# qasimyu/simuscop

Hardware: AMD Instinct MI355X
Metric: simulated paired reads/sec (whole node) at 30x WGS PE150 (higher is better)
Workload: dtype u32

## Files before the change

simuscop_amd/csrc/sg_api.cpp:

```cpp
#include <hip/hip_runtime.h>

#include <algorithm>
#include <chrono>
#include <cstdio>
#include <cstdlib>
#include <cstring>
#include <map>
#include <mutex>
#include <string>
#include <vector>

#include "sg_api.h"
#include "sg_deflate.h"
#include "sg_tables.h"
#include "sg_truth.h"

namespace {

struct BlockCache {
  struct Block { void* p; size_t cap; int dev; };
  std::mutex mu;
  std::vector<Block> blocks;
  size_t held = 0;
  static size_t limit() {
// ... 144 lines not shown
  int device = 0;
  hipStream_t stream = nullptr;
  DevBuf text[2], gz[2];
  uint64_t text_bytes[2] = {0, 0}, gz_bytes[2] = {0, 0};
  std::string err;
  ~sg_outputs() {
    if (stream) { (void)hipStreamSynchronize(stream); (void)hipStreamDestroy(stream); }
  }
};

sg_ctx::~sg_ctx() {
  (void)hipSetDevice(device);
  if (stream) (void)hipStreamSynchronize(stream);
  for (sg_outputs* o : spare) delete o;
  if (evs_created)
    for (auto& ev : evs) (void)hipEventDestroy(ev);
  if (own_stream) { (void)hipStreamSynchronize(own_stream); (void)hipStreamDestroy(own_stream); }
  if (mail) (void)hipHostFree(mail);
}

static int finish_plan(sg_ctx* ctx, uint64_t nw, uint32_t n_segs, uint32_t n_slots, uint32_t batch_id, uint32_t first_window,
                       uint32_t first_slot, int32_t paired, const char* name_prefix) {
  const size_t plen = name_prefix ? strlen(name_prefix) : 0;
  const uint32_t nm = paired ? 2 : 1;
  SG_ENSURE(ctx->prefix, plen + 16);
  SG_ENSURE(ctx->pairs, ((size_t)n_slots + 1) * sizeof(sg::PairRec));
  SG_ENSURE(ctx->win_actual, (nw + 1) * 4);
  SG_ENSURE(ctx->win_namebase, (nw + 1) * 4);
  SG_ENSURE(ctx->events, ((size_t)nm * n_slots + 1) * 4 * SG_MAX_EVENTS);
  SG_ENSURE(ctx->recoff, ((size_t)nm * n_slots + 1) * 4);
  SG_ENSURE(ctx->meta, ((size_t)nm * n_slots + 1) * 48);
  SG_ENSURE(ctx->totals, sg::kTotalsBytes);
  SG_ENSURE(ctx->bsum, ((size_t)nm * ((n_slots + 255) / 256) + 1) * 8);
  SG_HIP(hipMemcpyAsync(ctx->prefix.p, name_prefix, plen, hipMemcpyHostToDevice, ctx->stream));
  SG_HIP(hipStreamSynchronize(ctx->stream));

  sg::DevBatch& B = ctx->B;
  B.windows = ctx->windows.as<sg_window>();
  B.n_windows = nw;
  B.seg_size = ctx->segmeta.as<uint32_t>();
  B.seg_first_window = ctx->segmeta.as<uint32_t>() + n_segs;
  B.n_segs = n_segs;
  B.n_slots = n_slots;
  B.batch_id = batch_id;
  B.win_offset = first_window;
  B.slot_offset = first_slot;
  B.paired = paired ? 1 : 0;
  B.prefix = ctx->prefix.as<uint8_t>();
  B.prefix_len = (uint32_t)plen;
  for (int i = 0; i < 4; i++) B.prefix_w[i] = 0;
  for (size_t i = 0; i < plen && i < 16; i++) B.prefix_w[i / 4] |= (uint32_t)(uint8_t)name_prefix[i] << (8 * (i % 4));
  B.pairs = ctx->pairs.as<sg::PairRec>();
  B.win_actual = ctx->win_actual.as<uint32_t>();
  B.win_namebase = ctx->win_namebase.as<uint32_t>();
  B.events = ctx->events.as<uint32_t>();
  B.recloc = ctx->recoff.as<uint32_t>();
  B.blkbase = ctx->bsum.as<uint64_t>();
  B.seg_shift = sg::record_seg_shift((uint32_t)n_slots);
  B.meta = ctx->meta.as<uint4>();
  B.totals = ctx->totals.as<uint64_t>();
  B.slowq_count = (uint32_t*)(B.totals + 4);
  ctx->have_plan = true;
  ctx->sampled = false;
  ctx->results_valid = false;
  return SG_OK;
}

static int pack_chains(sg_ctx* ctx, size_t total) {
  const size_t q = total / 4, badb = total / 64 / 8;
  SG_ENSURE(ctx->chains2, 2 * q + badb + 64);
  uint8_t* p = ctx->chains2.as<uint8_t>();
  sg::launch_pack2(ctx->chains.as<uint8_t>(), total, (uint32_t*)p, (uint32_t*)(p + q), (uint16_t*)(p + 2 * q), ctx->stream);
  ctx->B.chains2_fwd = p;
  ctx->B.chains2_rc = p + q;
  ctx->B.chains_bad = (const uint16_t*)(p + 2 * q);
  ctx->B.chains_total = total;
  return SG_OK;
}

static sg_ctx::ChainLayout chain_layout(int32_t n_chains, const uint64_t* lens) {
  const size_t PAD = 256;
  sg_ctx::ChainLayout L;
  L.len.assign(lens, lens + n_chains);
  L.total = PAD;
  for (int c = 0; c < n_chains; c++) {
    L.off.push_back(L.total);
    L.total += (lens[c] + PAD + 63) & ~(size_t)63;
  }
  L.total = (L.total + PAD + 1023) & ~(size_t)1023;
  return L;
}

static int commit_chains(sg_ctx* ctx, sg_ctx::ChainLayout&& L) {
  std::vector<uint64_t> meta(L.off);
// ... 1010 lines not shown
  if (b->n_segs) {
    SG_HIP(hipMemcpyAsync(ctx->segmeta.p, b->seg_size, (size_t)b->n_segs * 4, hipMemcpyHostToDevice, ctx->stream));
    SG_HIP(hipMemcpyAsync(ctx->segmeta.as<uint32_t>() + b->n_segs, b->seg_first_window, ((size_t)b->n_segs + 1) * 4,
                          hipMemcpyHostToDevice, ctx->stream));
  }
  return finish_plan(ctx, nw, b->n_segs, (uint32_t)slots, b->batch_id, b->first_window, b->first_slot, b->paired, b->name_prefix);
}

static int launch_text(sg_ctx* ctx, bool prof) {
  sg::DevBatch& B = ctx->B;
  hipStream_t s = ctx->stream;
  B.out[0] = ctx->out1.as<uint8_t>();
  B.out[1] = ctx->out2.as<uint8_t>();
  B.out_cap[0] = ctx->out1.cap;
  B.out_cap[1] = ctx->out2.cap;
  B.slowq = nullptr;
  B.slowq_cap = 0;
  if (sg::emit_uses_fast_kernel(ctx->P, B)) {
    uint64_t cap = std::max<uint64_t>(1u << 16, 2ull * B.n_slots);
    if (const char* e = getenv("SG_SLOWQ_CAP")) cap = std::max<uint64_t>(1, strtoull(e, nullptr, 10));
    cap = std::min<uint64_t>(cap, 1ull << 30);
    SG_ENSURE(ctx->slowq, cap * 8 * (B.paired ? 2 : 1));
    B.slowq = ctx->slowq.as<uint2>();
    B.slowq_cap = (uint32_t)cap;
  }
  if (prof) SG_HIP(hipEventRecord(ctx->evs[5], s));
  sg::launch_header(ctx->P, B, s);
  ctx->emit_path = sg::emit_path(ctx->P, B, false);
  sg::launch_emit(ctx->P, B, s, false, prof ? ctx->evs[7] : nullptr);
  if (prof) SG_HIP(hipEventRecord(ctx->evs[6], s));
  return SG_OK;
}

static int run_pass(sg_ctx* ctx) {
  sg::DevBatch& B = ctx->B;
  B.k0 = (uint32_t)ctx->seed;
  B.k1 = (uint32_t)(ctx->seed >> 32);
  { const char* dg = getenv("SG_DIAG"); B.diag = dg ? (uint32_t)atoi(dg) : 0u; }
  if (const char* fd = getenv("SG_FDIAG")) B.diag = (uint32_t)atoi(fd);
  hipStream_t s = ctx->stream;
  const bool prof = ctx->profiling;
  if (!B.n_windows) SG_HIP(hipMemsetAsync(B.totals, 0, sg::kTotalsBytes, s));
  if (prof) SG_HIP(hipEventRecord(ctx->evs[0], s));
  sg::launch_plan(ctx->P, B, s);
  if (prof) SG_HIP(hipEventRecord(ctx->evs[1], s));
  sg::launch_namebase(B, s);
  if (prof) SG_HIP(hipEventRecord(ctx->evs[2], s));
  sg::launch_indel(ctx->P, B, s);
  if (prof) SG_HIP(hipEventRecord(ctx->evs[3], s));
  sg::launch_scan(B, s);
  if (prof) SG_HIP(hipEventRecord(ctx->evs[4], s));
  SG_HIP(hipGetLastError());
  if (!ctx->out1.p && !ctx->out2.p && !ctx->gz1.p && !ctx->gz2.p && !ctx->spare.empty()) {
    sg_outputs* o = ctx->spare.back();
    std::swap(ctx->out1, o->text[0]); std::swap(ctx->out2, o->text[1]);
    std::swap(ctx->gz1, o->gz[0]); std::swap(ctx->gz2, o->gz[1]);
  }
  ctx->speculative = ctx->out1.p != nullptr && (!B.paired || ctx->out2.p != nullptr) && getenv("SG_NO_SPECULATION") == nullptr;
  if (!ctx->speculative) {
    sg::launch_mail(B.totals, ctx->mail, s);
    SG_HIP(hipStreamSynchronize(s));
    memcpy(ctx->host_totals, ctx->mail, 4 * 8);
    if (ctx->host_totals[3] & 1) return ctx->fail(SG_ERR_OVERFLOW, "sg_sample: a read drew more than SG_MAX_EVENTS sequencing indels");
    SG_ENSURE(ctx->out1, ctx->host_totals[0] + 64);
    if (B.paired) SG_ENSURE(ctx->out2, ctx->host_totals[1] + 64);
  }
  if (int rc = launch_text(ctx, prof)) return rc;
  sg::launch_mail(B.totals, ctx->mail, s);
  SG_HIP(hipGetLastError());
  ctx->sampled = true;
  ctx->pass_pending = true;
  ctx->results_valid = false;
  ctx->gz_valid = false;
  return SG_OK;
}

static int finish_pass(sg_ctx* ctx) {
  if (!ctx->pass_pending) return SG_OK;
  SG_HIP(hipStreamSynchronize(ctx->stream));
  ctx->pass_pending = false;
  memcpy(ctx->host_totals, ctx->mail, 4 * 8);
// ... 350 lines not shown
```

simuscop_amd/csrc/sg_api.h:

```cpp
#pragma once
#include <hip/hip_runtime.h>

#include <map>
#include <string>
#include <utility>
#include <vector>

#include "sg_device.h"
#include "sg_haplotypes.h"

struct DevBuf {
  void* p = nullptr;
  size_t cap = 0;
  int dev = 0;
  DevBuf() = default;
  DevBuf(DevBuf&& o) noexcept : p(std::exchange(o.p, nullptr)), cap(std::exchange(o.cap, 0)), dev(o.dev) {}
  DevBuf& operator=(DevBuf&& o) noexcept {
    if (this != &o) { release(); p = std::exchange(o.p, nullptr); cap = std::exchange(o.cap, 0); dev = o.dev; }
    return *this;
  }
  DevBuf(const DevBuf&) = delete;
  DevBuf& operator=(const DevBuf&) = delete;
  ~DevBuf() { release(); }
  int ensure(size_t bytes);
  void release();
  template <class T> T* as() const { return (T*)p; }
};

extern thread_local std::string g_create_error;

struct sg_outputs;
struct sg_train_session;

struct sg_ctx {
  int device = 0;
  hipStream_t own_stream = nullptr;
  hipStream_t stream = nullptr;
  uint64_t seed = 0;
  std::string err;

  bool have_profile = false, have_haps = false, have_plan = false, sampled = false;
  sg::DevProfile P{};
  sg::DevBatch B{};
  DevBuf tab, chains, chains2, chain_meta, windows, segmeta, prefix, pairs, win_actual, win_namebase, events, recoff, meta, totals, bsum,
      out1, out2, gcw, gco, gcm, slowq, ref_raw, ref_codes, ref_meta, hap_work, gz1, gz2, gz_work,
      infl_src, infl_meta, infl_out, infl_crc,
      defl_src, defl_out;
  struct ChainLayout {
    std::vector<uint64_t> off, len;
    size_t total = 0;
  } hap;
  uint64_t gz_bytes[2] = {0, 0};
  bool gz_valid = false;
  struct Truth {
    uint64_t n_given = 0;
    bool from_build = false, mapped = false, valid = false;
    std::vector<sg_truth_piece> sorted;
    std::vector<uint64_t> chain_first;
    uint64_t rec_bytes = 0, gz_bytes = 0, records = 0, unmapped = 0;
  } truth;
  DevBuf truth_map, truth_work, truth_rec, truth_gz, truth_rows;
  struct Depth {
    bool on = false;
    std::vector<uint64_t> len, off;
    uint64_t slots = 0, m_bases = 0, scanned_starts = 0;
    int64_t scanned = -1;
  } depth;
  DevBuf depth_diff, depth_meta, depth_work, depth_out;
  struct Variants {
    bool on = false;
    uint64_t n = 0, reads_hit = 0, hits = 0;
  } variants;
  DevBuf var_rows, var_counts;
  std::vector<sg_outputs*> spare;
  std::map<uint32_t, DevBuf> wstore;
  std::map<uint32_t, uint64_t> wstore_n;
  DevBuf wplan, wwork;
  struct PlanInfo {
    bool valid = false;
    uint64_t n_windows = 0;
// ... 43 lines not shown
```

simuscop_amd/csrc/sg_device.h:

```cpp
#pragma once
#include <hip/hip_runtime.h>
#include <stdint.h>

#include "../../include/simuscop_amd.h"

namespace sg {

constexpr size_t kTotalsSegBase = 128 + 2 * 2 * 8 * 128;
constexpr size_t kTotalsBytes = kTotalsSegBase + 2 * 16 * 8 + 64;

constexpr int kBaseRounds = 7;

enum : uint32_t { KIND_HAP = 1, KIND_GC = 2, KIND_PLAN = 3, KIND_INDEL = 4, KIND_AUX = 5, KIND_BASE = 6 };

struct PairRec {
  uint32_t win;
  uint32_t namepos;
  uint32_t fl;
  uint32_t k;
  uint64_t foff;
  uint64_t pad;
};

__host__ __device__ inline uint32_t ev_pack(uint32_t j, uint32_t len, uint32_t del) { return j | (len << 16) | (del << 31); }
// ... 18 lines not shown
  int32_t L, bins, kmer, min_qual;
  uint32_t remap_packed;
  uint32_t bases_packed;
  uint32_t kmer_off[8];
  uint32_t inv_remap_packed;
};

struct DevBatch {
  const uint8_t* chains;
  const uint64_t* chain_off;
  const uint64_t* chain_len;
  const uint8_t* chains2_fwd;
  const uint8_t* chains2_rc;
  const uint16_t* chains_bad;
  uint64_t chains_total;
  const sg_window* windows;
  uint64_t n_windows;
  const uint32_t* seg_size;
  const uint32_t* seg_first_window;
  uint32_t n_segs;
  uint32_t n_slots;
  uint32_t batch_id;
  uint32_t win_offset, slot_offset;
  int32_t paired;
  const uint8_t* prefix;
  uint32_t prefix_len;
  uint32_t prefix_w[4];
  uint32_t k0, k1;
  uint32_t diag;
  uint32_t strict_bases;
  PairRec* pairs;
  uint32_t* win_actual;
  uint32_t* win_namebase;
  uint32_t* events;
  uint32_t* recloc;
  uint64_t* blkbase;
  uint32_t seg_shift;
  uint4* meta;
  uint64_t* totals;
  uint2* slowq;
  uint32_t* slowq_count;
  uint32_t slowq_cap;
  uint8_t* out[2];
  uint64_t out_cap[2];
};

void launch_plan(const DevProfile& P, const DevBatch& B, hipStream_t s);
void launch_namebase(const DevBatch& B, hipStream_t s);
void launch_indel(const DevProfile& P, const DevBatch& B, hipStream_t s);
void launch_scan(const DevBatch& B, hipStream_t s);
void launch_mail(const uint64_t* totals, uint64_t* mail, hipStream_t s);
void launch_header(const DevProfile& P, const DevBatch& B, hipStream_t s);
void launch_emit(const DevProfile& P, const DevBatch& B, hipStream_t s, bool force_generic, hipEvent_t after_main);
bool emit_uses_fast_kernel(const DevProfile& P, const DevBatch& B);
int emit_variant(const DevProfile& P);
struct EmitPath { int main_kernel; int slow_rows_lds; uint32_t lds_bytes, clean_cap; };
EmitPath emit_path(const DevProfile& P, const DevBatch& B, bool force_generic);
uint32_t record_seg_shift(uint32_t n_slots);
uint32_t scan_blocks(uint32_t n);
void launch_scan_u32(const uint32_t* in, uint32_t n, uint64_t* bsum, uint64_t* out, uint64_t* total, hipStream_t s);
void launch_encode(uint8_t* buf, size_t bytes, hipStream_t s);
void launch_gc(const uint8_t* chains, const uint64_t* chain_off, const sg_gc_window* wins, uint64_t n, int32_t* out, hipStream_t s);
void launch_tile(const sg_window_gen* gens, const uint64_t* prefix, uint32_t n_gens, uint64_t n, uint32_t frag, const uint64_t* seg_first,
                 sg_gc_window* out, uint32_t* seg_ord, uint32_t* win_ord, hipStream_t s);
void launch_seg_sum(const double* wt, const uint64_t* seg_first, uint32_t n_segs, double* out, hipStream_t s);
void launch_window_reads(const sg_window_gen* gens, const uint64_t* prefix, uint32_t n_gens, uint64_t n, uint32_t frag, const double* wt,
                         const sg_active_seg* act, const uint32_t* seg_first, uint32_t n_act, sg_window* rows, unsigned long long* seg_sum,
                         int32_t paired, uint32_t* planned, hipStream_t s);
void launch_slot_base(sg_window* rows, uint64_t n, const uint64_t* off, const uint32_t* seg_first, uint32_t n_act, const uint64_t* total,
                      uint64_t* seg_slots, hipStream_t s);
void launch_slice(const sg_window* all, uint64_t w_lo, uint64_t n, uint32_t a0, uint32_t slot_lo, sg_window* out, hipStream_t s);
void launch_gc_weight(const int32_t* gc, const sg_gc_window* wins, const uint32_t* seg_ord, const uint32_t* win_ord, uint64_t n,
                      const double* means, double std, const double* Q, uint32_t lg_cells, uint32_t frag, int32_t full_tile_form,
                      uint32_t ctx24, uint64_t seed, double* out, hipStream_t s);

}
```

simuscop_amd/csrc/sg_kernels.hip:

```cpp
#include <algorithm>
#include <cstdlib>
#include <type_traits>

#include "sg_device.h"

namespace sg {

template <int ROUNDS>
__device__ __forceinline__ void philox4x32(uint32_t c0, uint32_t c1, uint32_t c2, uint32_t c3,
                                           uint32_t k0, uint32_t k1, uint32_t out[4]) {
  const uint32_t M0 = 0xD2511F53u, M1 = 0xCD9E8D57u;
#pragma unroll
  for (int r = 0; r < ROUNDS; r++) {
    const uint64_t p0 = (uint64_t)M0 * c0, p1 = (uint64_t)M1 * c2;
    const uint32_t hi0 = (uint32_t)(p0 >> 32), lo0 = (uint32_t)p0;
    const uint32_t hi1 = (uint32_t)(p1 >> 32), lo1 = (uint32_t)p1;
    c0 = __builtin_amdgcn_bitop3_b32(hi1, c1, k0, 0x96);
    c1 = lo1;
    c2 = __builtin_amdgcn_bitop3_b32(hi0, c3, k1, 0x96);
    c3 = lo0;
    k0 += 0x9E3779B9u;
    k1 += 0xBB67AE85u;
  }
  out[0] = c0; out[1] = c1; out[2] = c2; out[3] = c3;
// ... 22 lines not shown
  philox4x32_10(slot + B.slot_offset, j, f >> 2, dev_ctx(KIND_AUX, mate, B.batch_id), B.k0, B.k1, x);
  uint32_t l = f & 3;
  return l == 0 ? x[0] : l == 1 ? x[1] : l == 2 ? x[2] : x[3];
}

__device__ __forceinline__ uint32_t ndigits(uint32_t v) {
  return v < 10 ? 1 : v < 100 ? 2 : v < 1000 ? 3 : v < 10000 ? 4 : v < 100000 ? 5 : v < 1000000 ? 6
       : v < 10000000 ? 7 : v < 100000000 ? 8 : v < 1000000000 ? 9 : 10;
}

#define PLAN_S 16

__device__ __forceinline__ bool plan_attempt(const DevProfile& P, const DevBatch& B, const sg_window& win, uint64_t w,
                                             uint32_t attempt, uint64_t clen, uint32_t c3, PairRec& r, const uint32_t* isz_row,
                                             uint32_t seg_size, uint64_t chain_off) {
  uint32_t x[4];
  philox4x32_10((uint32_t)w + B.win_offset, attempt, 0, c3, B.k0, B.k1, x);
  const double frac = __dmul_rn((double)x[0], 1.0 / 4294967296.0);
  const double v = __dadd_rn((double)win.spos, __dmul_rn((double)win.len, frac));
  const uint32_t pos = (uint32_t)(long long)v;
  uint32_t isz;
  if (B.paired) isz = isz_row ? (uint32_t)P.isz_min + row_search(isz_row, P.isz_lg, x[1]) : (uint32_t)P.fixed_isz;
  else isz = win.len;
  const uint64_t avail = clen - (win.hap_base + pos);
  const uint32_t flen = avail < (uint64_t)isz ? (uint32_t)avail : isz;
  const uint32_t strand = B.paired ? 0u : (x[2] >> 31);
  r.win = (uint32_t)w; r.fl = flen | (strand << 31);
  r.namepos = pos % seg_size;
  r.foff = chain_off + win.hap_base + pos;
  r.pad = 0;
  return flen >= (uint32_t)P.L;
}

__global__ __launch_bounds__(256) void plan_kernel(DevProfile P, DevBatch B) {
  __shared__ uint32_t isz_lds[1025];
  const uint32_t* isz_row = P.isz_row;
  if (P.isz_row && P.isz_lg <= 10u) {
    for (uint32_t i = threadIdx.x; i < (1u << P.isz_lg) + 1u; i += blockDim.x) isz_lds[i] = P.isz_row[i];
    isz_row = isz_lds;
  }
  __syncthreads();
  if (blockIdx.x == 0)
    for (uint32_t i = threadIdx.x; i < kTotalsBytes / 4u; i += blockDim.x) ((uint32_t*)B.totals)[i] = 0u;
  const uint64_t gid = (uint64_t)blockIdx.x * blockDim.x + threadIdx.x;
  const uint64_t w = gid / PLAN_S;
  const uint32_t j = (uint32_t)(gid % PLAN_S);
  if (w >= B.n_windows) return;
  const sg_window win = B.windows[w];
  const int n = win.n_reads;
  const uint32_t planned = n <= 0 ? 0u : (B.paired ? ((uint32_t)n + 1u) / 2u : (uint32_t)n);
  const uint64_t clen = B.chain_len[win.chain];
  const uint32_t seg_size = B.seg_size[win.seg];
  const uint64_t chain_off = B.chain_off[win.chain];
  const uint32_t c3 = dev_ctx(KIND_PLAN, 0, B.batch_id);
  const uint64_t last_start = win.hap_base + win.spos + win.len - 1u;
  const uint64_t need = B.paired ? (uint64_t)P.isz_hi : (uint64_t)win.len;
  const uint32_t shortest = B.paired ? (uint32_t)P.isz_lo : win.len;
  const bool safe = last_start + need <= clen && shortest >= (uint32_t)P.L;
  if (safe) {
    for (uint32_t k = j; k < planned; k += PLAN_S) {
      PairRec r;
      plan_attempt(P, B, win, w, k, clen, c3, r, isz_row, seg_size, chain_off);
      r.k = k;
      B.pairs[win.slot_base + k] = r;
    }
    if (j == 0) B.win_actual[w] = planned;
    return;
  }
  if (j != 0) return;
  uint32_t done = 0, fail = 0, attempt = 0;
  while (done < planned) {
    PairRec r;
    if (!plan_attempt(P, B, win, w, attempt++, clen, c3, r, isz_row, seg_size, chain_off)) {
      if (++fail > 1000) break;
      continue;
    }
    r.k = done;
    B.pairs[win.slot_base + done] = r;
    done++;
  }
  for (uint32_t k = done; k < planned; k++) {
    PairRec r;
    r.win = (uint32_t)w; r.namepos = 0; r.fl = 0; r.k = k; r.foff = 0; r.pad = 0;
    B.pairs[win.slot_base + k] = r;
  }
  B.win_actual[w] = done;
}

__global__ __launch_bounds__(64) void namebase_kernel(DevBatch B) {
  const uint32_t s = blockIdx.x;
  const uint32_t lane = threadIdx.x;
  const uint32_t w0 = B.seg_first_window[s], w1 = B.seg_first_window[s + 1];
  uint32_t carry = 0;
  for (uint32_t base = w0; base < w1; base += 64) {
    uint32_t w = base + lane;
    uint32_t v = w < w1 ? B.win_actual[w] : 0u;
    uint32_t incl = v;
#pragma unroll
    for (int d = 1; d < 64; d <<= 1) {
      uint32_t t = __shfl_up(incl, d);
      if ((int)lane >= d) incl += t;
    }
    if (w < w1) B.win_namebase[w] = carry + incl - v;
    carry += __shfl(incl, 63);
  }
  if (lane == 0) atomicAdd((unsigned long long*)&B.totals[2], (unsigned long long)carry);
}

__device__ __forceinline__ void wave_lds_sync() {
  __builtin_amdgcn_fence(__ATOMIC_RELEASE, "wavefront");
  __builtin_amdgcn_wave_barrier();
  __builtin_amdgcn_fence(__ATOMIC_ACQUIRE, "wavefront");
}

__device__ __forceinline__ uint64_t rec_offset(const DevBatch& B, uint32_t m, uint32_t t) {
  const uint32_t blk = t >> 8;
  const uint64_t* segbase = (const uint64_t*)((const uint8_t*)B.totals + kTotalsSegBase);
  return segbase[m * 16u + (blk >> B.seg_shift)] + B.blkbase[(size_t)m * ((B.n_slots + 255u) >> 8) + blk] +
         B.recloc[(size_t)m * B.n_slots + t];
}

__global__ __launch_bounds__(256) void indel_kernel(DevProfile P, DevBatch B) {
  __shared__ uint4 row_lds[256 * 3];
  __shared__ uint16_t cand[512];
  __shared__ uint32_t cand_n;
  __shared__ uint2 found[2][256];
  __shared__ uint32_t found_first[2][256];
  __shared__ uint32_t wave_len[2][4];
  const uint32_t tid = threadIdx.x, lane = tid & 63u, wv = tid >> 6;
  const uint32_t t = blockIdx.x * blockDim.x + tid;
  const uint32_t nm = B.paired ? 2u : 1u;
  uint4* const wave_rows = row_lds + (tid & ~63u) * 3u;
  uint4* const my_row = wave_rows + lane * 3u;
  const uint32_t t_wave = t - lane;
  __shared__ uint64_t gap_lds[256];
  const uint64_t* gap = P.gap_row;
  if ((uint32_t)P.L + 1u <= 256u) {
    for (uint32_t i = tid; i <= (uint32_t)P.L; i += blockDim.x) gap_lds[i] = P.gap_row[i];
    gap = gap_lds;
  }
  if (tid == 0u) cand_n = 0u;
  const bool in_batch = t < B.n_slots;
  PairRec rec = {};
  if (in_batch) rec = B.pairs[t];
  const uint32_t flen = rec.fl & 0x7FFFFFFFu;
  const bool live = flen != 0u;
  const uint32_t L = (uint32_t)P.L;
  uint32_t fragcount = 0, touches_bad[2] = {0, 0};
  const uint64_t foff = rec.foff;
  const uint32_t rev1 = rec.fl >> 31;
  if (live) {
    fragcount = B.win_namebase[rec.win] + rec.k + 1u;
    for (uint32_t m = 0; m < nm; m++) {
      const bool rev = B.paired ? (m == 1u) : (rev1 != 0u);
      const uint64_t t0 = (rev ? foff + flen - L : foff) - 8u, t1 = t0 + L + 24u;
      uint32_t bad = 0;
      for (uint64_t b = t0 >> 6; b <= (t1 >> 6); b++) bad |= (B.chains_bad[b >> 4] >> (b & 15u)) & 1u;
      touches_bad[m] = bad;
    }
  }
  __syncthreads();
  for (uint32_t m = 0; m < nm; m++) {
    found[m][tid] = make_uint2(0u, 0u);
    found_first[m][tid] = 0u;
    bool has = false;
    if (live) {
      uint32_t x4[4];
      philox4x32_10(t + B.slot_offset, 0u, 0, dev_ctx(KIND_INDEL, m, B.batch_id), B.k0, B.k1, x4);
      const uint64_t x = ((uint64_t)x4[1] << 32) | x4[0];
      has = !(x < gap[L]);
    }
    const unsigned long long hm = __ballot(has);
    if (hm) {
      uint32_t base = 0;
      if (lane == (uint32_t)__builtin_ctzll(hm)) base = atomicAdd(&cand_n, (uint32_t)__popcll(hm));
      base = __shfl(base, __builtin_ctzll(hm), 64);
      if (has) cand[base + (uint32_t)__popcll(hm & ((1ull << lane) - 1ull))] = (uint16_t)(tid | (m << 8));
    }
  }
  __syncthreads();
  {
    const uint32_t nc = cand_n;
#pragma unroll 1
    for (uint32_t i = tid; i < nc; i += blockDim.x) {
      const uint32_t e16 = cand[i], lt = e16 & 255u, m = e16 >> 8;
      const uint32_t tt = blockIdx.x * blockDim.x + lt;
      uint32_t* ev = B.events + ((size_t)m * B.n_slots + tt) * SG_MAX_EVENTS;
      const uint32_t c3 = dev_ctx(KIND_INDEL, m, B.batch_id);
      int j = 0, dl = 0;
      uint32_t nev = 0, first_ev = 0, e = 0;
#pragma unroll 1
      while (j < (int)L) {
        uint32_t x4[4];
        philox4x32_10(tt + B.slot_offset, e++, 0, c3, B.k0, B.k1, x4);
        const uint64_t x = ((uint64_t)x4[1] << 32) | x4[0], y = ((uint64_t)x4[3] << 32) | x4[2];
        const int room = (int)L - j;
        if (x < gap[room]) break;
        int lo = 0, hi = room - 1;
        while (lo < hi) {
          const int mid = (lo + hi + 1) >> 1;
          if (x < gap[mid]) lo = mid; else hi = mid - 1;
        }
        const int jj = j + lo;
        const bool is_ins = __umul64hi(y, P.evB) < P.evA;
        j = jj + 1;
        if (is_ins) {
          uint32_t len = row_search(P.ins_row, P.ins_lg, aux_draw(B, tt, (uint32_t)jj, 0, m));
          if (len > 0) {
            if (nev < SG_MAX_EVENTS) ev[nev] = ev_pack((uint32_t)jj, len, 0);
            if (nev == 0) first_ev = ev_pack((uint32_t)jj, len, 0);
            nev++;
            dl += (int)len;
          }
        } else {
          uint32_t len = row_search(P.del_row, P.del_lg, aux_draw(B, tt, (uint32_t)jj, 0, m));
          if (len > 0) {
            uint32_t k = min((uint32_t)((int)L - jj), len);
            if (nev < SG_MAX_EVENTS) ev[nev] = ev_pack((uint32_t)jj, k, 1);
            if (nev == 0) first_ev = ev_pack((uint32_t)jj, k, 1);
            nev++;
            dl -= (int)k;
            j = jj + (int)k;
          }
        }
      }
      found[m][lt] = make_uint2(nev, (uint32_t)dl);
      found_first[m][lt] = first_ev;
    }
  }
  __syncthreads();
  const uint32_t namepos = rec.namepos;
  const uint32_t hdr = B.prefix_len + ndigits(namepos) + 1u + ndigits(fragcount) + (B.paired ? 2u : 0u) + 1u;
  uint32_t mate_at = 0;
  my_row[0] = live ? make_uint4((uint32_t)foff, (uint32_t)(foff >> 32), namepos, fragcount) : make_uint4(0, 0, 0, 0);
  my_row[2] = make_uint4(0, 0, 0, 0);
  if (live && hdr - B.prefix_len <= 16u) {
    uint8_t* hb = (uint8_t*)(my_row + 2);
    uint32_t o = 0;
    auto put_dec = [&](uint32_t v) {
      const uint32_t nd = ndigits(v);
      for (uint32_t k = nd; k-- > 0u;) {
        const uint32_t qd = v / 10u;
        hb[o + k] = (uint8_t)('0' + (v - qd * 10u));
        v = qd;
      }
      o += nd;
    };
    put_dec(namepos);
// ... 25 lines not shown
    if (t_wave < B.n_slots) {
      wave_lds_sync();
      uint4* dst = B.meta + ((size_t)m * B.n_slots + t_wave) * 3;
      const uint32_t n_pieces = min(B.n_slots - t_wave, 64u) * 3u;
#pragma unroll
      for (uint32_t i = 0; i < 3u; i++) {
        const uint32_t q = i * 64u + lane;
        if (q < n_pieces) dst[q] = wave_rows[q];
      }
    }
  }
  uint32_t incl[2];
  for (uint32_t m = 0; m < nm; m++) {
    uint32_t v = rl[m];
#pragma unroll
    for (int d = 1; d < 64; d <<= 1) {
      const uint32_t up = __shfl_up(v, d, 64);
      if ((int)lane >= d) v += up;
    }
    incl[m] = v;
    if (lane == 63u) wave_len[m][wv] = v;
  }
  __syncthreads();
  for (uint32_t m = 0; m < nm; m++) {
    uint32_t base = 0, all = 0;
#pragma unroll
    for (uint32_t i = 0; i < 4u; i++) {
      const uint32_t w = wave_len[m][i];
      if (i < wv) base += w;
      all += w;
    }
    if (in_batch) B.recloc[(size_t)m * B.n_slots + t] = base + incl[m] - rl[m];
    if (tid == 0u) B.blkbase[(size_t)m * gridDim.x + blockIdx.x] = all;
  }
}

__device__ __attribute__((noinline)) void write_name(uint8_t* hp, const uint8_t* __restrict__ prefix, uint32_t prefix_len,
                                                     uint32_t namepos, uint32_t fragcount, uint32_t paired, uint32_t m) {
  uint32_t w = 0, nb = 0;
  auto push = [&](uint32_t b) {
    w |= b << (nb * 8u);
    if (++nb == 4u) { __builtin_memcpy(hp, &w, 4); hp += 4; w = 0; nb = 0; }
  };
  auto push_dec = [&](uint32_t v) {
    const uint32_t nd = ndigits(v);
    uint64_t lo = 0;
    uint32_t hi = 0;
    for (uint32_t k = 0; k < nd; k++) {
      const uint32_t qd = v / 10u, d = '0' + (v - qd * 10u);
      if (k < 8u) lo = (lo << 8) | d; else hi = (hi << 8) | d;
      v = qd;
    }
    for (uint32_t k = 8; k < nd; k++) { push(hi & 0xFFu); hi >>= 8; }
    for (uint32_t k = 0; k < (nd < 8u ? nd : 8u); k++) { push((uint32_t)lo & 0xFFu); lo >>= 8; }
  };
  for (uint32_t i = 0; i < prefix_len; i++) push(prefix[i]);
  push_dec(namepos);
  push('#');
  push_dec(fragcount);
  if (paired) { push('/'); push('1' + m); }
  push('\n');
  for (uint32_t i = 0; i < nb; i++) hp[i] = (uint8_t)(w >> (8u * i));
}

__global__ __launch_bounds__(256) void header_kernel(DevBatch B) {
  const uint32_t t = blockIdx.x * blockDim.x + threadIdx.x;
// ... 1521 lines not shown
  if (w >= n) return;
  const int32_t r = rows[w].n_reads;
  planned[w] = r <= 0 ? 0u : (paired ? ((uint32_t)r + 1u) / 2u : (uint32_t)r);
}
__global__ __launch_bounds__(256) void slot_base_kernel(sg_window* __restrict__ rows, uint64_t n, const uint64_t* __restrict__ off) {
  const uint64_t w = (uint64_t)blockIdx.x * blockDim.x + threadIdx.x;
  if (w < n) rows[w].slot_base = (uint32_t)off[w];
}
__global__ __launch_bounds__(64) void seg_slots_kernel(const uint64_t* __restrict__ off, const uint32_t* __restrict__ seg_first, uint32_t n_act,
                                                       const uint64_t* __restrict__ total, uint64_t* __restrict__ out) {
  const uint32_t a = blockIdx.x * blockDim.x + threadIdx.x;
  if (a < n_act) out[a] = off[seg_first[a]];
  if (a == n_act) out[a] = *total;
}
__global__ __launch_bounds__(256) void slice_kernel(const sg_window* __restrict__ all, uint64_t w_lo, uint64_t n, uint32_t a0, uint32_t slot_lo,
                                                    sg_window* __restrict__ out) {
  const uint64_t w = (uint64_t)blockIdx.x * blockDim.x + threadIdx.x;
  if (w >= n) return;
  sg_window o = all[w_lo + w];
  o.seg -= a0;
  o.slot_base -= slot_lo;
  out[w] = o;
}

__global__ void mail_kernel(const uint64_t* __restrict__ totals, uint64_t* __restrict__ mail) {
  if (threadIdx.x < 5u) mail[threadIdx.x] = totals[threadIdx.x];
}
void launch_mail(const uint64_t* totals, uint64_t* mail, hipStream_t s) {
  hipLaunchKernelGGL(mail_kernel, dim3(1), dim3(64), 0, s, totals, mail);
}
void launch_plan(const DevProfile& P, const DevBatch& B, hipStream_t s) {
  if (!B.n_windows) return;
  uint32_t grid = (uint32_t)((B.n_windows * PLAN_S + 255) / 256);
  hipLaunchKernelGGL(plan_kernel, dim3(grid), dim3(256), 0, s, P, B);
}
void launch_namebase(const DevBatch& B, hipStream_t s) {
  if (!B.n_segs) return;
  hipLaunchKernelGGL(namebase_kernel, dim3(B.n_segs), dim3(64), 0, s, B);
}
void launch_indel(const DevProfile& P, const DevBatch& B, hipStream_t s) {
  if (!B.n_slots) return;
  hipLaunchKernelGGL(indel_kernel, dim3((B.n_slots + 255) / 256), dim3(256), 0, s, P, B);
}
void launch_header(const DevProfile& P, const DevBatch& B, hipStream_t s) {
  if (!B.n_slots) return;
  const bool fast = emit_uses_fast_kernel(P, B);
  if (fast && B.prefix_len <= 16u) return;
  dim3 grid((B.n_slots + 255) / 256, B.paired ? 2 : 1);
  hipLaunchKernelGGL(header_kernel, grid, dim3(256), 0, s, B);
}
uint32_t scan_blocks(uint32_t n) { return (n + SCAN_TILE - 1) / SCAN_TILE; }
uint32_t record_seg_shift(uint32_t n_slots) {
  const uint32_t nblk = (n_slots + 255u) >> 8;
  uint32_t k = 0;
  while (((nblk + (1u << k) - 1u) >> k) > 16u) k++;
  return k;
}
void launch_scan(const DevBatch& B, hipStream_t s) {
  if (!B.n_slots) return;
  hipLaunchKernelGGL(block_base_kernel, dim3(16, B.paired ? 2 : 1), dim3(1024), 0, s, B);
}
void launch_scan_u32(const uint32_t* in, uint32_t n, uint64_t* bsum, uint64_t* out, uint64_t* total, hipStream_t s) {
  if (!n) return;
  const uint32_t nblk = scan_blocks(n);
  hipLaunchKernelGGL(scan_reduce_kernel, dim3(nblk, 1), dim3(SCAN_BLOCK), 0, s, in, n, bsum, nblk);
  hipLaunchKernelGGL(scan_sums_kernel, dim3(1), dim3(1024), 0, s, bsum, nblk, total);
  hipLaunchKernelGGL(scan_apply_kernel, dim3(nblk, 1), dim3(SCAN_BLOCK), 0, s, in, n, bsum, nblk, out);
}
static const size_t kLdsBytes = 160 * 1024;
template <int KT, bool SL>
static void launch_emit_variant(const DevProfile& P, const DevBatch& B, dim3 grid, size_t lds, uint32_t sub_rows, uint32_t TI,
                                uint32_t RPI, hipStream_t s) {
  (void)hipFuncSetAttribute((const void*)emit_kernel<KT, SL>, hipFuncAttributeMaxDynamicSharedMemorySize, (int)lds);
  hipLaunchKernelGGL((emit_kernel<KT, SL>), grid, dim3(EMIT_THREADS), lds, s, P, B, sub_rows, TI, RPI);
}
// ... 147 lines not shown
```

simuscop_amd/csrc/sg_truth.h:

```cpp
#pragma once
#include <hip/hip_runtime.h>
#include <stdint.h>

#include "sg_device.h"

namespace sg {

enum : uint32_t { kOpM = 0, kOpI = 1, kOpD = 2, kOpN = 3, kOpS = 4 };

struct TruthPiece {
  uint64_t dst;
  uint64_t src;
  uint32_t len;
  uint32_t meta;
};
__host__ __device__ inline uint32_t truth_meta(uint32_t contig, uint32_t kind, uint32_t seg_first) {
  return (contig & 0x3FFFFFFFu) | ((kind ? 1u : 0u) << 30) | ((seg_first ? 1u : 0u) << 31);
}

struct TruthAln {
  int32_t contig;
  int64_t pos0, end;
  uint32_t n_ops;
};
// ... 102 lines not shown
  return lo;
}

__host__ __device__ inline uint32_t truth_reg2bin(int64_t beg, int64_t end) {
  --end;
  if (beg >> 14 == end >> 14) return (uint32_t)(((1 << 15) - 1) / 7 + (beg >> 14));
  if (beg >> 17 == end >> 17) return (uint32_t)(((1 << 12) - 1) / 7 + (beg >> 17));
  if (beg >> 20 == end >> 20) return (uint32_t)(((1 << 9) - 1) / 7 + (beg >> 20));
  if (beg >> 23 == end >> 23) return (uint32_t)(((1 << 6) - 1) / 7 + (beg >> 23));
  if (beg >> 26 == end >> 26) return (uint32_t)(((1 << 3) - 1) / 7 + (beg >> 26));
  return 0;
}

struct ReadGeom {
  bool live, inside;
  uint32_t chain, reverse, np, nev, hdr;
  uint64_t tmpl_off;
  const uint32_t* events;
};
__device__ __forceinline__ ReadGeom read_geom(const DevProfile& P, const DevBatch& B, uint32_t t, uint32_t m) {
  ReadGeom g = {};
  const size_t idx = (size_t)m * B.n_slots + t;
  const uint4 m1 = B.meta[idx * 3 + 1];
  const uint32_t flen = m1.x & 0x3FFFFFFFu;
  g.live = flen != 0u;
  if (!g.live) return g;
  const uint4 m0 = B.meta[idx * 3];
  const uint64_t foff = ((uint64_t)m0.y << 32) | m0.x;
  const uint32_t L = (uint32_t)P.L;
  g.reverse = m1.x >> 31;
  g.np = m1.y & 0xFFFFu;
  g.nev = (m1.y >> 16) & 63u;
  g.hdr = m1.y >> 22;
  g.chain = B.windows[B.pairs[t].win].chain;
  const uint64_t c0 = B.chain_off[g.chain], tmpl = g.reverse ? foff + flen - L : foff;
  g.inside = flen >= L && tmpl >= c0 && tmpl - c0 + L <= B.chain_len[g.chain];
  g.tmpl_off = tmpl - c0;
  g.events = B.events + idx * SG_MAX_EVENTS;
  return g;
}

constexpr uint32_t kTruthMaxOps = 256;
constexpr uint32_t kTruthWaveOps = 2048;

struct TruthRow {
  int32_t contig;
  int32_t pos, end;
  uint32_t n_ops;
};

struct TruthJob {
  const TruthPiece* pieces;
  const uint64_t* chain_first;
  uint32_t n_chains;
  uint32_t n_reads;
  TruthRow* rows;
  uint32_t* rec_len;
  const uint64_t* rec_off;
  unsigned long long* counters;
  uint8_t* out;
  uint64_t out_bytes;
  uint32_t text_lds;
  uint32_t image_lds;
};
void launch_truth_size(const DevProfile& P, const DevBatch& B, const TruthJob& J, hipStream_t s);
void launch_truth_pack(const DevProfile& P, const DevBatch& B, const TruthJob& J, hipStream_t s);
struct TruthReadRow {
// ... 128 lines not shown
```

Before: 2.146 billion.

## Precompute static window plan and fuse safe-window draws into fragment kernel

Moves the per-batch window classification (safe vs tail windows, slot-to-window map, name bases) into a one-time static pass at plan time. The per-pass front end then runs only a small tail-planning kernel for windows near chain ends, and draws fragment pairs for safe windows directly inside the indel kernel, dropping the separate plan and namebase launches and the PairRec round-trip through global memory. Indel and deletion length rows are also staged in LDS. This adds a sync at plan time and depends on the safe-window criterion exactly matching the retry logic of the original planner. Truth geometry now reads window ids from the new slot map.

Result: faster. 2.191 billion, median of 6 (+2.1%).

```diff
diff --git a/simuscop_amd/csrc/sg_api.cpp b/simuscop_amd/csrc/sg_api.cpp
--- a/simuscop_amd/csrc/sg_api.cpp
+++ b/simuscop_amd/csrc/sg_api.cpp
@@ -200,8 +200,11 @@
   SG_ENSURE(ctx->meta, ((size_t)nm * n_slots + 1) * 48);
   SG_ENSURE(ctx->totals, sg::kTotalsBytes);
   SG_ENSURE(ctx->bsum, ((size_t)nm * ((n_slots + 255) / 256) + 1) * 8);
+  if (!ctx->have_haps) return ctx->fail(SG_ERR_INVALID, "sg_plan: call sg_upload_haplotypes first");
+  if (nw > 0x7FFFFFFFull) return ctx->fail(SG_ERR_INVALID, "sg_plan: more than 2^31 windows in one batch");
+  const size_t o_slot = 16, o_tw = o_slot + ((size_t)n_slots + 1) * 4, o_seg = o_tw + (nw + 1) * 4, seg_b = ((size_t)n_segs + 1) * 4;
+  SG_ENSURE(ctx->front, o_seg + 5 * seg_b);
   SG_HIP(hipMemcpyAsync(ctx->prefix.p, name_prefix, plen, hipMemcpyHostToDevice, ctx->stream));
-  SG_HIP(hipStreamSynchronize(ctx->stream));
 
   sg::DevBatch& B = ctx->B;
   B.windows = ctx->windows.as<sg_window>();
@@ -228,6 +231,23 @@
   B.meta = ctx->meta.as<uint4>();
   B.totals = ctx->totals.as<uint64_t>();
   B.slowq_count = (uint32_t*)(B.totals + 4);
+  {
+    uint8_t* f = ctx->front.as<uint8_t>();
+    uint32_t* segs = (uint32_t*)(f + o_seg);
+    const uint32_t ns1 = n_segs + 1;
+    sg::launch_front_static(ctx->P, B, (uint32_t*)(f + o_slot), (uint32_t*)(f + o_tw), segs, segs + ns1, segs + 2 * ns1, (uint64_t*)f, ctx->stream);
+    SG_HIP(hipGetLastError());
+    uint64_t hdr[2] = {0, 0};
+    SG_HIP(hipMemcpyAsync(hdr, f, 16, hipMemcpyDeviceToHost, ctx->stream));
+    SG_HIP(hipStreamSynchronize(ctx->stream));
+    B.front_hdr = (const uint64_t*)f;
+    B.slot_win = (const uint32_t*)(f + o_slot);
+    B.tail_wins = (const uint32_t*)(f + o_tw);
+    B.seg_tail_n = segs;
+    B.tail_segs = segs + 2 * ns1;
+    B.seg_short = segs + 3 * ns1;
+    B.n_tail_segs = (uint32_t)hdr[1];
+  }
   ctx->have_plan = true;
   ctx->sampled = false;
   ctx->results_valid = false;
@@ -1304,6 +1324,8 @@
   return SG_OK;
 }
 
+static bool env_is(const char* v, char c) { return v != nullptr && v[0] == c && v[1] == 0; }
+
 static int run_pass(sg_ctx* ctx) {
   sg::DevBatch& B = ctx->B;
   B.k0 = (uint32_t)ctx->seed;
@@ -1312,13 +1334,23 @@
   if (const char* fd = getenv("SG_FDIAG")) B.diag = (uint32_t)atoi(fd);
   hipStream_t s = ctx->stream;
   const bool prof = ctx->profiling;
-  if (!B.n_windows) SG_HIP(hipMemsetAsync(B.totals, 0, sg::kTotalsBytes, s));
-  if (prof) SG_HIP(hipEventRecord(ctx->evs[0], s));
-  sg::launch_plan(ctx->P, B, s);
-  if (prof) SG_HIP(hipEventRecord(ctx->evs[1], s));
-  sg::launch_namebase(B, s);
-  if (prof) SG_HIP(hipEventRecord(ctx->evs[2], s));
-  sg::launch_indel(ctx->P, B, s);
+  const bool legacy = env_is(getenv("SG_LEGACY_FRONT"), '1');
+  if (legacy) {
+    if (!B.n_windows) SG_HIP(hipMemsetAsync(B.totals, 0, sg::kTotalsBytes, s));
+    if (prof) SG_HIP(hipEventRecord(ctx->evs[0], s));
+    sg::launch_plan(ctx->P, B, s);
+    if (prof) SG_HIP(hipEventRecord(ctx->evs[1], s));
+    sg::launch_namebase(B, s);
+    if (prof) SG_HIP(hipEventRecord(ctx->evs[2], s));
+    sg::launch_indel(ctx->P, B, s);
+  } else {
+    const bool draws = !env_is(getenv("SG_FRONT_DRAWS"), '0'), rows = !env_is(getenv("SG_FRONT_ROWS"), '0');
+    if (prof) SG_HIP(hipEventRecord(ctx->evs[0], s));
+    sg::launch_plan_tail(ctx->P, B, draws, s);
+    if (prof) SG_HIP(hipEventRecord(ctx->evs[1], s));
+    if (prof) SG_HIP(hipEventRecord(ctx->evs[2], s));
+    sg::launch_fragment(ctx->P, B, draws, rows, s);
+  }
   if (prof) SG_HIP(hipEventRecord(ctx->evs[3], s));
   sg::launch_scan(B, s);
   if (prof) SG_HIP(hipEventRecord(ctx->evs[4], s));
diff --git a/simuscop_amd/csrc/sg_api.h b/simuscop_amd/csrc/sg_api.h
--- a/simuscop_amd/csrc/sg_api.h
+++ b/simuscop_amd/csrc/sg_api.h
@@ -45,7 +45,8 @@
   DevBuf tab, chains, chains2, chain_meta, windows, segmeta, prefix, pairs, win_actual, win_namebase, events, recoff, meta, totals, bsum,
       out1, out2, gcw, gco, gcm, slowq, ref_raw, ref_codes, ref_meta, hap_work, gz1, gz2, gz_work,
       infl_src, infl_meta, infl_out, infl_crc,
-      defl_src, defl_out;
+      defl_src, defl_out,
+      front;
   struct ChainLayout {
     std::vector<uint64_t> off, len;
     size_t total = 0;
diff --git a/simuscop_amd/csrc/sg_device.h b/simuscop_amd/csrc/sg_device.h
--- a/simuscop_amd/csrc/sg_device.h
+++ b/simuscop_amd/csrc/sg_device.h
@@ -74,6 +74,13 @@
   PairRec* pairs;
   uint32_t* win_actual;
   uint32_t* win_namebase;
+  const uint32_t* slot_win;
+  const uint32_t* tail_wins;
+  const uint32_t* seg_tail_n;
+  const uint32_t* tail_segs;
+  uint32_t n_tail_segs;
+  uint32_t* seg_short;
+  const uint64_t* front_hdr;
   uint32_t* events;
   uint32_t* recloc;
   uint64_t* blkbase;
@@ -90,6 +97,10 @@
 void launch_plan(const DevProfile& P, const DevBatch& B, hipStream_t s);
 void launch_namebase(const DevBatch& B, hipStream_t s);
 void launch_indel(const DevProfile& P, const DevBatch& B, hipStream_t s);
+void launch_front_static(const DevProfile& P, const DevBatch& B, uint32_t* slot_win, uint32_t* tail_wins, uint32_t* seg_tail_n,
+                         uint32_t* seg_planned, uint32_t* tail_segs, uint64_t* hdr, hipStream_t s);
+void launch_plan_tail(const DevProfile& P, const DevBatch& B, bool draws, hipStream_t s);
+void launch_fragment(const DevProfile& P, const DevBatch& B, bool draws, bool rows, hipStream_t s);
 void launch_scan(const DevBatch& B, hipStream_t s);
 void launch_mail(const uint64_t* totals, uint64_t* mail, hipStream_t s);
 void launch_header(const DevProfile& P, const DevBatch& B, hipStream_t s);
diff --git a/simuscop_amd/csrc/sg_kernels.hip b/simuscop_amd/csrc/sg_kernels.hip
--- a/simuscop_amd/csrc/sg_kernels.hip
+++ b/simuscop_amd/csrc/sg_kernels.hip
@@ -78,6 +78,7 @@
   return flen >= (uint32_t)P.L;
 }
 
+template <bool SAFE_ONLY>
 __global__ __launch_bounds__(256) void plan_kernel(DevProfile P, DevBatch B) {
   __shared__ uint32_t isz_lds[1025];
   const uint32_t* isz_row = P.isz_row;
@@ -86,7 +87,7 @@
     isz_row = isz_lds;
   }
   __syncthreads();
-  if (blockIdx.x == 0)
+  if (!SAFE_ONLY && blockIdx.x == 0)
     for (uint32_t i = threadIdx.x; i < kTotalsBytes / 4u; i += blockDim.x) ((uint32_t*)B.totals)[i] = 0u;
   const uint64_t gid = (uint64_t)blockIdx.x * blockDim.x + threadIdx.x;
   const uint64_t w = gid / PLAN_S;
@@ -110,10 +111,10 @@
       r.k = k;
       B.pairs[win.slot_base + k] = r;
     }
-    if (j == 0) B.win_actual[w] = planned;
+    if (!SAFE_ONLY && j == 0) B.win_actual[w] = planned;
     return;
   }
-  if (j != 0) return;
+  if (SAFE_ONLY || j != 0) return;
   uint32_t done = 0, fail = 0, attempt = 0;
   while (done < planned) {
     PairRec r;
@@ -153,6 +154,150 @@
   if (lane == 0) atomicAdd((unsigned long long*)&B.totals[2], (unsigned long long)carry);
 }
 
+__device__ __forceinline__ uint32_t window_planned(const DevBatch& B, const sg_window& win) {
+  const int n = win.n_reads;
+  return n <= 0 ? 0u : (B.paired ? ((uint32_t)n + 1u) / 2u : (uint32_t)n);
+}
+__device__ __forceinline__ bool window_safe(const DevProfile& P, const DevBatch& B, const sg_window& win) {
+  const uint64_t clen = B.chain_len[win.chain];
+  const uint64_t last_start = win.hap_base + win.spos + win.len - 1u;
+  const uint64_t need = B.paired ? (uint64_t)P.isz_hi : (uint64_t)win.len;
+  const uint32_t shortest = B.paired ? (uint32_t)P.isz_lo : win.len;
+  return last_start + need <= clen && shortest >= (uint32_t)P.L;
+}
+
+__global__ __launch_bounds__(256) void slot_map_kernel(DevProfile P, DevBatch B, uint32_t* __restrict__ slot_win) {
+  const uint64_t gid = (uint64_t)blockIdx.x * blockDim.x + threadIdx.x;
+  const uint64_t w = gid / PLAN_S;
+  const uint32_t j = (uint32_t)(gid % PLAN_S);
+  if (w >= B.n_windows) return;
+  const sg_window win = B.windows[w];
+  const uint32_t planned = window_planned(B, win);
+  const uint32_t v = (uint32_t)w | (window_safe(P, B, win) ? 0u : 0x80000000u);
+  for (uint32_t k = j; k < planned; k += PLAN_S) slot_win[win.slot_base + k] = v;
+}
+
+__global__ __launch_bounds__(64) void seg_static_kernel(DevProfile P, DevBatch B, uint32_t* __restrict__ tail_wins,
+                                                        uint32_t* __restrict__ seg_tail_n, uint32_t* __restrict__ seg_planned) {
+  const uint32_t s = blockIdx.x;
+  const uint32_t lane = threadIdx.x;
+  const uint32_t w0 = B.seg_first_window[s], w1 = B.seg_first_window[s + 1];
+  uint32_t carry = 0, ntail = 0;
+  for (uint32_t base = w0; base < w1; base += 64) {
+    const uint32_t w = base + lane;
+    uint32_t v = 0;
+    bool tail = false;
+    if (w < w1) {
+      const sg_window win = B.windows[w];
+      v = window_planned(B, win);
+      tail = v != 0u && !window_safe(P, B, win);
+      B.win_actual[w] = v;
+    }
+    uint32_t incl = v;
+#pragma unroll
+    for (int d = 1; d < 64; d <<= 1) {
+      uint32_t t = __shfl_up(incl, d);
+      if ((int)lane >= d) incl += t;
+    }
+    if (w < w1) B.win_namebase[w] = carry + incl - v;
+    carry += __shfl(incl, 63);
+    const unsigned long long tm = __ballot(tail);
+    if (tail) tail_wins[w0 + ntail + (uint32_t)__popcll(tm & ((1ull << lane) - 1ull))] = w;
+    ntail += (uint32_t)__popcll(tm);
+  }
+  if (lane == 0) { seg_tail_n[s] = ntail; seg_planned[s] = carry; }
+}
+
+__global__ __launch_bounds__(64) void tail_segs_kernel(const uint32_t* __restrict__ seg_tail_n, const uint32_t* __restrict__ seg_planned,
+                                                       uint32_t n_segs, uint32_t* __restrict__ tail_segs, uint64_t* __restrict__ hdr) {
+  const uint32_t lane = threadIdx.x;
+  uint32_t cnt = 0;
+  uint64_t total = 0;
+  for (uint32_t base = 0; base < n_segs; base += 64) {
+    const uint32_t s = base + lane;
+    const bool has = s < n_segs && seg_tail_n[s] != 0u;
+    total += s < n_segs ? seg_planned[s] : 0u;
+    const unsigned long long hm = __ballot(has);
+    if (has) tail_segs[cnt + (uint32_t)__popcll(hm & ((1ull << lane) - 1ull))] = s;
+    cnt += (uint32_t)__popcll(hm);
+  }
+#pragma unroll
+  for (int d = 32; d >= 1; d >>= 1) total += __shfl_xor(total, d);
+  if (lane == 0) { hdr[0] = total; hdr[1] = cnt; }
+}
+
+__global__ __launch_bounds__(256) void plan_tail_kernel(DevProfile P, DevBatch B) {
+  __shared__ uint32_t isz_lds[1025];
+  __shared__ uint32_t short_sum;
+  const uint32_t tid = threadIdx.x, lane = tid & 63u, wv = tid >> 6;
+  const uint32_t* isz_row = P.isz_row;
+  if (P.isz_row && P.isz_lg <= 10u) {
+    for (uint32_t i = tid; i < (1u << P.isz_lg) + 1u; i += blockDim.x) isz_lds[i] = P.isz_row[i];
+    isz_row = isz_lds;
+  }
+  if (tid == 0u) short_sum = 0u;
+  __syncthreads();
+  if (blockIdx.x == 0)
+    for (uint32_t i = tid; i < kTotalsBytes / 4u; i += blockDim.x) ((uint32_t*)B.totals)[i] = 0u;
+  if (blockIdx.x >= B.n_tail_segs) return;
+  const uint32_t s = B.tail_segs[blockIdx.x];
+  const uint32_t w0 = B.seg_first_window[s], w1 = B.seg_first_window[s + 1];
+  const uint32_t nt = B.seg_tail_n[s];
+  const uint32_t c3 = dev_ctx(KIND_PLAN, 0, B.batch_id);
+  const unsigned long long upto = lane == 63u ? ~0ull : ((2ull << lane) - 1ull);
+  for (uint32_t i = wv; i < nt; i += 4u) {
+    const uint32_t w = B.tail_wins[w0 + i];
+    const sg_window win = B.windows[w];
+    const uint32_t planned = window_planned(B, win);
+    const uint64_t clen = B.chain_len[win.chain];
+    const uint32_t seg_size = B.seg_size[win.seg];
+    const uint64_t chain_off = B.chain_off[win.chain];
+    uint32_t done = 0, fail = 0, base = 0;
+    while (done < planned && fail <= 1000u) {
+      PairRec r;
+      const bool ok = plan_attempt(P, B, win, w, base + lane, clen, c3, r, isz_row, seg_size, chain_off);
+      const unsigned long long succ = __ballot(ok);
+      const uint32_t rs = (uint32_t)__popcll(succ & upto), rf = (uint32_t)__popcll(~succ & upto);
+      const unsigned long long endm = __ballot(ok ? rs == planned - done : rf == 1001u - fail);
+      const uint32_t cut = endm ? (uint32_t)__builtin_ctzll(endm) : 63u;
+      const unsigned long long counted = cut == 63u ? ~0ull : ((2ull << cut) - 1ull);
+      if (ok && lane <= cut) {
+        r.k = done + rs - 1u;
+        B.pairs[win.slot_base + r.k] = r;
+      }
+      done += (uint32_t)__popcll(succ & counted);
+      fail += (uint32_t)__popcll(~succ & counted);
+      base += 64u;
+    }
+    for (uint32_t k = done + lane; k < planned; k += 64u) {
+      PairRec r;
+      r.win = w; r.namepos = 0; r.fl = 0; r.k = k; r.foff = 0; r.pad = 0;
+      B.pairs[win.slot_base + k] = r;
+    }
+    if (lane == 0u) {
+      B.win_actual[w] = done;
+      atomicAdd(&short_sum, planned - done);
+    }
+  }
+  __threadfence_block();
+  __syncthreads();
+  if (tid == 0u) B.seg_short[blockIdx.x] = short_sum;
+  if (wv != 0u) return;
+  uint32_t carry = 0;
+  for (uint32_t base = w0; base < w1; base += 64) {
+    const uint32_t w = base + lane;
+    const uint32_t v = w < w1 ? B.win_actual[w] : 0u;
+    uint32_t incl = v;
+#pragma unroll
+    for (int d = 1; d < 64; d <<= 1) {
+      uint32_t t = __shfl_up(incl, d);
+      if ((int)lane >= d) incl += t;
+    }
+    if (w < w1) B.win_namebase[w] = carry + incl - v;
+    carry += __shfl(incl, 63);
+  }
+}
+
 __device__ __forceinline__ void wave_lds_sync() {
   __builtin_amdgcn_fence(__ATOMIC_RELEASE, "wavefront");
   __builtin_amdgcn_wave_barrier();
@@ -166,6 +311,9 @@
          B.recloc[(size_t)m * B.n_slots + t];
 }
 
+enum : int { FRONT_TAIL = 1, FRONT_DRAWS = 2, FRONT_ROWS = 4 };
+constexpr uint32_t kLenRowCap = 257;
+template <int MODE>
 __global__ __launch_bounds__(256) void indel_kernel(DevProfile P, DevBatch B) {
   __shared__ uint4 row_lds[256 * 3];
   __shared__ uint16_t cand[512];
@@ -187,8 +335,43 @@
   }
   if (tid == 0u) cand_n = 0u;
   const bool in_batch = t < B.n_slots;
+  uint32_t* const stage = (uint32_t*)row_lds;
+  const uint32_t* ins_row = P.ins_row;
+  const uint32_t* del_row = P.del_row;
+  if constexpr ((MODE & FRONT_ROWS) != 0) {
+    if ((1u << P.ins_lg) + 1u <= kLenRowCap && (1u << P.del_lg) + 1u <= kLenRowCap) {
+      for (uint32_t i = tid; i < (1u << P.ins_lg) + 1u; i += blockDim.x) stage[1025u + i] = P.ins_row[i];
+      for (uint32_t i = tid; i < (1u << P.del_lg) + 1u; i += blockDim.x) stage[1025u + kLenRowCap + i] = P.del_row[i];
+      ins_row = stage + 1025u;
+      del_row = stage + 1025u + kLenRowCap;
+    }
+  }
   PairRec rec = {};
-  if (in_batch) rec = B.pairs[t];
+  uint32_t namebase = 0;
+  if constexpr ((MODE & FRONT_DRAWS) != 0) {
+    const uint32_t* isz_row = P.isz_row;
+    if (B.paired && P.isz_row && P.isz_lg <= 10u) {
+      for (uint32_t i = tid; i < (1u << P.isz_lg) + 1u; i += blockDim.x) stage[i] = P.isz_row[i];
+      isz_row = stage;
+    }
+    sg_window win = {};
+    uint32_t sw = 0x80000000u, seg_size = 1u;
+    uint64_t chain_off = 0;
+    if (in_batch) {
+      sw = B.slot_win[t];
+      win = B.windows[sw & 0x7FFFFFFFu];
+      namebase = B.win_namebase[sw & 0x7FFFFFFFu];
+      if (sw >> 31) rec = B.pairs[t];
+      else { seg_size = B.seg_size[win.seg]; chain_off = B.chain_off[win.chain]; }
+    }
+    __syncthreads();
+    if (!(sw >> 31)) {
+      plan_attempt(P, B, win, sw, t - win.slot_base, ~0ull, dev_ctx(KIND_PLAN, 0, B.batch_id), rec, isz_row, seg_size, chain_off);
+      rec.k = t - win.slot_base;
+    }
+  } else {
+    if (in_batch) rec = B.pairs[t];
+  }
   const uint32_t flen = rec.fl & 0x7FFFFFFFu;
   const bool live = flen != 0u;
   const uint32_t L = (uint32_t)P.L;
@@ -196,7 +379,8 @@
   const uint64_t foff = rec.foff;
   const uint32_t rev1 = rec.fl >> 31;
   if (live) {
-    fragcount = B.win_namebase[rec.win] + rec.k + 1u;
+    if constexpr ((MODE & FRONT_DRAWS) == 0) namebase = B.win_namebase[rec.win];
+    fragcount = namebase + rec.k + 1u;
     for (uint32_t m = 0; m < nm; m++) {
       const bool rev = B.paired ? (m == 1u) : (rev1 != 0u);
       const uint64_t t0 = (rev ? foff + flen - L : foff) - 8u, t1 = t0 + L + 24u;
@@ -205,7 +389,7 @@
       touches_bad[m] = bad;
     }
   }
-  __syncthreads();
+  if constexpr ((MODE & FRONT_DRAWS) == 0) __syncthreads();
   for (uint32_t m = 0; m < nm; m++) {
     found[m][tid] = make_uint2(0u, 0u);
     found_first[m][tid] = 0u;
@@ -251,7 +435,7 @@
         const bool is_ins = __umul64hi(y, P.evB) < P.evA;
         j = jj + 1;
         if (is_ins) {
-          uint32_t len = row_search(P.ins_row, P.ins_lg, aux_draw(B, tt, (uint32_t)jj, 0, m));
+          uint32_t len = row_search(ins_row, P.ins_lg, aux_draw(B, tt, (uint32_t)jj, 0, m));
           if (len > 0) {
             if (nev < SG_MAX_EVENTS) ev[nev] = ev_pack((uint32_t)jj, len, 0);
             if (nev == 0) first_ev = ev_pack((uint32_t)jj, len, 0);
@@ -259,7 +443,7 @@
             dl += (int)len;
           }
         } else {
-          uint32_t len = row_search(P.del_row, P.del_lg, aux_draw(B, tt, (uint32_t)jj, 0, m));
+          uint32_t len = row_search(del_row, P.del_lg, aux_draw(B, tt, (uint32_t)jj, 0, m));
           if (len > 0) {
             uint32_t k = min((uint32_t)((int)L - jj), len);
             if (nev < SG_MAX_EVENTS) ev[nev] = ev_pack((uint32_t)jj, k, 1);
@@ -351,6 +535,15 @@
     }
     if (in_batch) B.recloc[(size_t)m * B.n_slots + t] = base + incl[m] - rl[m];
     if (tid == 0u) B.blkbase[(size_t)m * gridDim.x + blockIdx.x] = all;
+  }
+  if constexpr ((MODE & FRONT_TAIL) != 0) {
+    if (blockIdx.x == 0u && wv == 0u) {
+      uint64_t lack = 0;
+      for (uint32_t i = lane; i < B.n_tail_segs; i += 64u) lack += B.seg_short[i];
+#pragma unroll
+      for (int d = 32; d >= 1; d >>= 1) lack += __shfl_xor(lack, d);
+      if (lane == 0u) B.totals[2] = B.front_hdr[0] - lack;
+    }
   }
 }
 
@@ -1938,7 +2131,7 @@
 void launch_plan(const DevProfile& P, const DevBatch& B, hipStream_t s) {
   if (!B.n_windows) return;
   uint32_t grid = (uint32_t)((B.n_windows * PLAN_S + 255) / 256);
-  hipLaunchKernelGGL(plan_kernel, dim3(grid), dim3(256), 0, s, P, B);
+  hipLaunchKernelGGL(plan_kernel<false>, dim3(grid), dim3(256), 0, s, P, B);
 }
 void launch_namebase(const DevBatch& B, hipStream_t s) {
   if (!B.n_segs) return;
@@ -1946,7 +2139,31 @@
 }
 void launch_indel(const DevProfile& P, const DevBatch& B, hipStream_t s) {
   if (!B.n_slots) return;
-  hipLaunchKernelGGL(indel_kernel, dim3((B.n_slots + 255) / 256), dim3(256), 0, s, P, B);
+  hipLaunchKernelGGL(indel_kernel<0>, dim3((B.n_slots + 255) / 256), dim3(256), 0, s, P, B);
+}
+void launch_front_static(const DevProfile& P, const DevBatch& B, uint32_t* slot_win, uint32_t* tail_wins, uint32_t* seg_tail_n,
+                         uint32_t* seg_planned, uint32_t* tail_segs, uint64_t* hdr, hipStream_t s) {
+  if (B.n_windows) {
+    const uint32_t grid = (uint32_t)((B.n_windows * PLAN_S + 255) / 256);
+    hipLaunchKernelGGL(slot_map_kernel, dim3(grid), dim3(256), 0, s, P, B, slot_win);
+  }
+  if (B.n_segs) hipLaunchKernelGGL(seg_static_kernel, dim3(B.n_segs), dim3(64), 0, s, P, B, tail_wins, seg_tail_n, seg_planned);
+  hipLaunchKernelGGL(tail_segs_kernel, dim3(1), dim3(64), 0, s, seg_tail_n, seg_planned, B.n_segs, tail_segs, hdr);
+}
+void launch_plan_tail(const DevProfile& P, const DevBatch& B, bool draws, hipStream_t s) {
+  hipLaunchKernelGGL(plan_tail_kernel, dim3(std::max(1u, B.n_tail_segs)), dim3(256), 0, s, P, B);
+  if (!draws && B.n_windows) {
+    const uint32_t grid = (uint32_t)((B.n_windows * PLAN_S + 255) / 256);
+    hipLaunchKernelGGL(plan_kernel<true>, dim3(grid), dim3(256), 0, s, P, B);
+  }
+}
+void launch_fragment(const DevProfile& P, const DevBatch& B, bool draws, bool rows, hipStream_t s) {
+  if (!B.n_slots) return;
+  const dim3 grid((B.n_slots + 255) / 256), block(256);
+  if (draws && rows) hipLaunchKernelGGL(indel_kernel<FRONT_TAIL | FRONT_DRAWS | FRONT_ROWS>, grid, block, 0, s, P, B);
+  else if (draws) hipLaunchKernelGGL(indel_kernel<FRONT_TAIL | FRONT_DRAWS>, grid, block, 0, s, P, B);
+  else if (rows) hipLaunchKernelGGL(indel_kernel<FRONT_TAIL | FRONT_ROWS>, grid, block, 0, s, P, B);
+  else hipLaunchKernelGGL(indel_kernel<FRONT_TAIL>, grid, block, 0, s, P, B);
 }
 void launch_header(const DevProfile& P, const DevBatch& B, hipStream_t s) {
   if (!B.n_slots) return;
diff --git a/simuscop_amd/csrc/sg_truth.h b/simuscop_amd/csrc/sg_truth.h
--- a/simuscop_amd/csrc/sg_truth.h
+++ b/simuscop_amd/csrc/sg_truth.h
@@ -158,7 +158,7 @@
   g.np = m1.y & 0xFFFFu;
   g.nev = (m1.y >> 16) & 63u;
   g.hdr = m1.y >> 22;
-  g.chain = B.windows[B.pairs[t].win].chain;
+  g.chain = B.windows[B.slot_win[t] & 0x7FFFFFFFu].chain;
   const uint64_t c0 = B.chain_off[g.chain], tmpl = g.reverse ? foff + flen - L : foff;
   g.inside = flen >= L && tmpl >= c0 && tmpl - c0 + L <= B.chain_len[g.chain];
   g.tmpl_off = tmpl - c0;
```
